# eduard-permyakov/permafrost-engine

Hardware: AMD Instinct MI355X
Metric: agent-steps/sec (+ flow-field cells/sec), every chunk field rebuilt + every agent stepped per tick (higher is better)
Workload: dtype u64-bitmask/u8 fields, f32 agents (f64 exp); 1 GPU; BASELINE configs[2]: 1024x1024 cells, 64 flow fields = 16384 chunk fields, 100000 agents; map_chunks=16, flow_fields=64, agents=100000, hz=20, dynamic_obstacles=0, parallelism=requests by destination + uid slabs x1, 1 all-gather (16 B/agent) per tick, ranks=1, rccl_ranks=1, backend=none, tile_exchange=auto, requests=reference planner fixture, has_dest_los=device lookup, initial_velocities=flow aligned, fields_ahead=True, tick_driver=c (navhip_tick_run), library=libnavhip.so (in-tree)

## Files before the change

permafrost-engine_amd/csrc/field_kernels.hip:

```cpp
#include "navhip_internal.h"

#include "wave_bits.h"

__device__ __forceinline__ bool req_uses_bfs(const nh_map_view &map, const navhip_field_req &rq,
                                             int force_generic)
{
    if(force_generic) return false;
    if(rq.type == NAVHIP_TARGET_NEAREST_PATHABLE || (rq.flags & NAVHIP_REQ_ISLAND_NEAREST)) return false;
    const nh_layer_view &L = map.layers[rq.layer];
    return L.unit_cost[(int)rq.chunk_r * map.w + rq.chunk_c] != 0;
}

__device__ __forceinline__ uint16_t portal_first_iid(const uint16_t *li, int r0, int c0, int r1, int c1)
{
    for(int r = r0; r <= r1; r++)
        for(int c = c0; c <= c1; c++) {
            const uint16_t v = li[r * 64 + c];
            if(v != NAVHIP_ISLAND_NONE) return v;
        }
    return NAVHIP_ISLAND_NONE;
}

__device__ __forceinline__ bool req_prepare(const nh_map_view &map, navhip_field_req &rq)
{
    const nh_layer_view &L = map.layers[rq.layer];
    const bool portal = rq.type == NAVHIP_TARGET_PORTAL;
    if((rq.flags & NAVHIP_REQ_IF_CHANGED) && L.changed) {
        bool ch = L.changed[(int)rq.chunk_r * map.w + rq.chunk_c] != 0;
        if(portal) ch |= L.changed[(int)rq.next_chunk_r * map.w + rq.next_chunk_c] != 0;
        if(rq.faction_id != NAVHIP_FACTION_ID_NONE && L.fac_changed)
            ch |= (L.fac_changed[(int)rq.chunk_r * map.w + rq.chunk_c] & ~rq.enemies & 0x7fff) != 0;
        if(!ch) return false;
    }
    if((rq.flags & NAVHIP_REQ_LIVE_IIDS) && portal && L.local_islands) {
        rq.port_iid = portal_first_iid(L.local_islands + ((size_t)((int)rq.chunk_r * map.w + rq.chunk_c) << 12),
                                       rq.port_r0, rq.port_c0, rq.port_r1, rq.port_c1);
        rq.next_iid = portal_first_iid(L.local_islands + ((size_t)((int)rq.next_chunk_r * map.w + rq.next_chunk_c) << 12),
                                       rq.next_r0, rq.next_c0, rq.next_r1, rq.next_c1);
        if(rq.port_iid == NAVHIP_ISLAND_NONE || rq.next_iid == NAVHIP_ISLAND_NONE) return false;
    }
    return true;
}

__device__ __forceinline__ bool next_tile_matches(const nh_map_view &map, const navhip_field_req &rq,
                                                  int gr, int gc)
{
    if(gr < 0 || gc < 0) return false;
    int cr2 = gr >> 6, cc2 = gc >> 6, r2 = gr & 63, c2 = gc & 63;
    if(cr2 != rq.next_chunk_r || cc2 != rq.next_chunk_c) return false;
    if(cr2 >= map.h || cc2 >= map.w) return false;
    if(r2 < rq.next_r0 || r2 > rq.next_r1 || c2 < rq.next_c0 || c2 > rq.next_c1) return false;
    const uint16_t *li = map.layers[rq.layer].local_islands;
    return li[((size_t)(cr2 * map.w + cc2) << 12) + r2 * 64 + c2] == rq.next_iid;
}

__device__ __forceinline__ bool portal_seed(const nh_map_view &map, const navhip_field_req &rq,
                                            int r, int c, bool passable)
{
    if(!passable) return false;
    if(r < rq.port_r0 || r > rq.port_r1 || c < rq.port_c0 || c > rq.port_c1) return false;
    const uint16_t *li = map.layers[rq.layer].local_islands;
    size_t cbase = (size_t)((int)rq.chunk_r * map.w + rq.chunk_c) << 12;
    if(rq.port_iid != NAVHIP_ISLAND_NONE && li[cbase + r * 64 + c] != rq.port_iid) return false;
    int gr = rq.chunk_r * 64 + r, gc = rq.chunk_c * 64 + c;
    return next_tile_matches(map, rq, gr - 1, gc) || next_tile_matches(map, rq, gr + 1, gc)
        || next_tile_matches(map, rq, gr, gc - 1) || next_tile_matches(map, rq, gr, gc + 1);
}

__device__ __forceinline__ uint32_t portal_fix_dir(const navhip_field_req &rq)
{
    if(rq.next_chunk_r < rq.chunk_r) return NAVHIP_FD_N;
    if(rq.next_chunk_r > rq.chunk_r) return NAVHIP_FD_S;
    if(rq.next_chunk_c < rq.chunk_c) return NAVHIP_FD_W;
    return NAVHIP_FD_E;
}

__global__ __launch_bounds__(256) void k_derive(const uint8_t *cost, const uint16_t *blockers,
                                                uint64_t *passmask, uint64_t *probemask, uint8_t *unit_cost,
                                                const uint8_t *factions, uint64_t *facmask, uint16_t *facany,
                                                const uint32_t *chunk_list, int n)
{
    int wave = (blockIdx.x * 256 + threadIdx.x) >> 6;
    int lane = threadIdx.x & 63;
    if(wave >= n) return;
    uint32_t chunk = chunk_list ? chunk_list[wave] : (uint32_t)wave;
    const uint8_t  *cb = cost + ((size_t)chunk << 12);
    const uint16_t *bl = blockers ? blockers + ((size_t)chunk << 12) : nullptr;
    uint64_t mine = 0, path = 0, blocked = 0;
    bool nonunit = false;
    for(int r = 0; r < 64; r++) {
        uint32_t cst = cb[r * 64 + lane];
        uint32_t blk = bl ? bl[r * 64 + lane] : 0;
        uint64_t m = __ballot(cst != NAVHIP_COST_IMPASSABLE && blk == 0);
        uint64_t mp = __ballot(cst != NAVHIP_COST_IMPASSABLE), mb = __ballot(blk > 0);
        nonunit |= (cst != NAVHIP_COST_IMPASSABLE && cst != 1);
        if(lane == r) { mine = m; path = mp; blocked = mb; }
    }
    passmask[(size_t)chunk * 64 + lane] = mine;
    probemask[((size_t)chunk * 64 + lane) * 2]     = path;
    probemask[((size_t)chunk * 64 + lane) * 2 + 1] = blocked;
    bool any_nonunit = __any(nonunit);
    if(lane == 0) unit_cost[chunk] = any_nonunit ? 0 : 1;
    if(factions) {
        const uint8_t *fa = factions + ((size_t)chunk * NAVHIP_MAX_FACTIONS << 12) + lane * 64;
        uint32_t any = 0;
        for(int f = 0; f < NAVHIP_MAX_FACTIONS; f++) {
            const uint64_t m = nz_row_mask(fa + ((size_t)f << 12));
            facmask[((size_t)chunk * NAVHIP_MAX_FACTIONS + f) * 64 + lane] = m;
            if(__ballot(m != 0)) any |= 1u << f;
        }
        if(lane == 0) facany[chunk] = (uint16_t)any;
    }
}

void nh_launch_derive(navhip_ctx *ctx, int layer, const uint32_t *d_chunk_list, int n, hipStream_t s)
{
    navhip_layer &L = ctx->layers[layer];
    int blocks = (n + 3) / 4;
    hipLaunchKernelGGL(k_derive, dim3(blocks), dim3(256), 0, s, L.cost, L.blockers, L.passmask, L.probemask,
                       L.unit_cost, L.factions, L.facmask, L.facany, d_chunk_list, n);
}

__device__ __forceinline__ uint64_t faction_pass_row(const nh_layer_view &L, int chunk, int lane, uint32_t enemies)
{
    const uint64_t *pm = L.probemask + ((size_t)chunk * 64 + lane) * 2;
    const uint64_t path = pm[0], blocked = pm[1];
    if(!L.facmask) return path;
    uint64_t friends = 0;
    uint32_t fs = __builtin_amdgcn_readfirstlane((int)(L.facany[chunk] & ~enemies & ((1u << NAVHIP_MAX_FACTIONS) - 1u)));
    const uint64_t *fm = L.facmask + (size_t)chunk * NAVHIP_MAX_FACTIONS * 64 + lane;
    while(fs) {
        const int f = __builtin_ctz(fs);
        fs &= fs - 1;
        friends |= fm[f * 64];
    }
    return path & ~(blocked & friends);
}

#define NH_MAXP 12
#define BFS_WAVES 4

template <bool WANT_INTEG>
__global__ __launch_bounds__(BFS_WAVES * 64) void k_field_bfs(nh_map_view map, const navhip_field_req *reqs,
                                                   int n, uint8_t *dirs, float *integ,
                                                   int force_generic, int32_t *gen_list, int gen_slot,
                                                   const int32_t *out_slot)
{
    __shared__ __attribute__((aligned(16))) uint8_t stage[BFS_WAVES][NH_CELLS];

    const int wib  = threadIdx.x >> 6;
    const int wave = blockIdx.x * BFS_WAVES + wib;
    const int lane = threadIdx.x & 63;
    if(wave >= n) return;

    navhip_field_req rq = reqs[wave];
    if(!req_uses_bfs(map, rq, force_generic)) {
        if(lane == 0) gen_list[2 + atomicAdd(&gen_list[gen_slot], 1)] = wave;
        return;
    }
    if(!req_prepare(map, rq)) return;

    const nh_layer_view &L = map.layers[rq.layer];
    const int chunk = (int)rq.chunk_r * map.w + rq.chunk_c;
    const u64x pass = mk(rq.faction_id == NAVHIP_FACTION_ID_NONE ? L.passmask[(size_t)chunk * 64 + lane]
                                                                 : faction_pass_row(L, chunk, lane, rq.enemies));

    u64x seeds = u64x{0, 0};
    if(rq.type == NAVHIP_TARGET_TILE) {
        if(lane == rq.tile_r) seeds = mk(1ull << rq.tile_c) & pass;
    }else{
        if(rq.port_c0 == rq.port_c1) {
            bool s = portal_seed(map, rq, lane, rq.port_c0, (to64(pass) >> rq.port_c0) & 1);
            if(s) seeds = mk(1ull << rq.port_c0);
        }else{
            for(int r = rq.port_r0; r <= rq.port_r1; r++) {
                uint64_t prow = __shfl(to64(pass), r);
                bool s = portal_seed(map, rq, r, lane, (prow >> lane) & 1);
                uint64_t m = __ballot(s);
                if(lane == r) seeds = mk(m);
            }
        }
    }

    u64x open = andn(pass, seeds);
    u64x frontier = seeds;
    u64x pl[NH_MAXP];
#pragma unroll
    for(int k = 0; k < NH_MAXP; k++) pl[k] = u64x{0, 0};

    int level = 0;
#define NH_BFS_LEVEL(NLOW)                                                                   \
    {                                                                                        \
        u64x nw = bfs_reach(frontier, open);                                                 \
        if(!__any(nz(nw))) break;                                                            \
        level++;                                                                             \
        pl[0] = pl[0] ^ open;                                                                \
        if(NLOW > 1) pl[1] = pl[1] ^ open;                                                   \
        if(NLOW > 2) pl[2] = pl[2] ^ open;                                                   \
        if(NLOW > 3) {                                                                       \
            const int tz = __builtin_ctz(level);          \
            _Pragma("unroll")                                                                \
            for(int k = 3; k < NH_MAXP; k++) {                                               \
                if(k <= tz) pl[k] = pl[k] ^ open;                                            \
            }                                                                                \
        }                                                                                    \
        open = andn(open, nw);                                                               \
        frontier = nw;                                                                       \
    }
    for(;;) {
        NH_BFS_LEVEL(1) NH_BFS_LEVEL(2) NH_BFS_LEVEL(1) NH_BFS_LEVEL(3)
        NH_BFS_LEVEL(1) NH_BFS_LEVEL(2) NH_BFS_LEVEL(1) NH_BFS_LEVEL(4)
    }
#undef NH_BFS_LEVEL
    const u64x reach = andn(pass, open);
#pragma unroll
    for(int k = 0; k < NH_MAXP; k++) pl[k] = pl[k] & reach;

    const int P = 32 - __builtin_clz((unsigned)level + 1);

    if(WANT_INTEG) {
        float *out = integ + ((size_t)wave << 12);
        for(int c = 0; c < 64; c++) {
            uint32_t d = 0;
#pragma unroll
            for(int k = 0; k < NH_MAXP; k++) d |= (uint32_t)((to64(pl[k]) >> c) & 1) << k;
            bool fin = (to64(reach) >> c) & 1;
            out[lane * 64 + c] = fin ? (float)d : __builtin_inff();
        }
    }

    u64x anybit = u64x{0, 0};
#pragma unroll
    for(int k = 0; k < NH_MAXP; k++) anybit = anybit | pl[k];
    const u64x zero = andn(reach, anybit);
    const u64x act  = reach & anybit;

    const u64x rN = from_n(reach), rS = from_s(reach), rW = from_w(reach), rE = from_e(reach);
    u64x eqN, eqS, eqW, eqE;
    {
        const u64x m0 = pl[0], m1 = pl[1];
        u64x n0, n1;
        n0 = from_n(pl[0]); n1 = from_n(pl[1]); eqN = andn(n0 ^ m0, n1 ^ n0 ^ m1) & rN;
        n0 = from_s(pl[0]); n1 = from_s(pl[1]); eqS = andn(n0 ^ m0, n1 ^ n0 ^ m1) & rS;
        n0 = from_w(pl[0]); n1 = from_w(pl[1]); eqW = andn(n0 ^ m0, n1 ^ n0 ^ m1) & rW;
        n0 = from_e(pl[0]); n1 = from_e(pl[1]); eqE = andn(n0 ^ m0, n1 ^ n0 ^ m1) & rE;
    }

    u64x neNW = u64x{0, 0}, neNE = neNW, neSW = neNW, neSE = neNW;
    {
        u64x b1 = u64x{~0u, ~0u};
        u64x b2 = u64x{~0u, ~0u};
#pragma unroll
        for(int k = 0; k < NH_MAXP; k++) {
            if(k < P) {
                u64x e = pl[k] ^ b1;  b1 = andn(b1, pl[k]);
                u64x f = e ^ b2;      b2 = andn(b2, e);
                u64x up = from_n(pl[k]), dn = from_s(pl[k]);
                neNW = neNW | (from_w(up) ^ f);
                neNE = neNE | (from_e(up) ^ f);
                neSW = neSW | (from_w(dn) ^ f);
                neSE = neSE | (from_e(dn) ^ f);
            }
        }
    }
    const u64x eqNW = andn(from_w(rN), neNW), eqNE = andn(from_e(rN), neNE);
    const u64x eqSW = andn(from_w(rS), neSW), eqSE = andn(from_e(rS), neSE);

    const u64x hasD = (eqNW & rN & rW) | (eqNE & rN & rE) | (eqSW & rS & rW) | (eqSE & rS & rE);
    const u64x h = act & hasD;
    const u64x g = andn(act, hasD);

    const u64x mN  = g & eqN;
    const u64x mS  = andn(g & eqS, eqN);
    const u64x mE  = andn(g & eqE, eqN | eqS);
    const u64x mW  = andn(g & eqW, eqN | eqS | eqE);
    const u64x mNW = h & eqNW;
    const u64x mNE = andn(h & eqNE, eqNW);
    const u64x mSW = andn(h & eqSW, eqNW | eqNE);
    const u64x mSE = andn(h & eqSE, eqNW | eqNE | eqSW);

    u64x D0 = mNW | mNE | mE | mS;
    u64x D1 = mN | mNE | mSW | mS;
    u64x D2 = mW | mE | mSW | mS;
    u64x D3 = mSE;
    if(rq.type == NAVHIP_TARGET_PORTAL) {
        uint32_t fd = portal_fix_dir(rq);
        if(fd & 1) D0 = D0 | zero;
        if(fd & 2) D1 = D1 | zero;
        if(fd & 4) D2 = D2 | zero;
    }

    uint8_t *out = dirs + ((size_t)(out_slot ? out_slot[wave] : wave) << 12);
    uint8_t *st = stage[wib];
    const bool inout = (rq.flags & NAVHIP_REQ_INOUT) != 0;
    if(inout) {
#pragma unroll
        for(int j = 0; j < 4; j++)
            *(uint4*)(st + j * 1024 + lane * 16) = *(const uint4*)(out + j * 1024 + lane * 16);
    }
    __builtin_amdgcn_wave_barrier();
    {
        uint32_t *row = (uint32_t*)(st + lane * 64);
        const uint64_t d0 = to64(D0), d1 = to64(D1), d2 = to64(D2), d3 = to64(D3);
        const uint64_t rc = to64(reach);
#pragma unroll
        for(int j = 0; j < 16; j++) {
            uint32_t b0 = (((uint32_t)(d0 >> (4 * j)) & 0xf) * 0x00204081u) & 0x01010101u;
            uint32_t b1 = (((uint32_t)(d1 >> (4 * j)) & 0xf) * 0x00204081u) & 0x01010101u;
            uint32_t b2 = (((uint32_t)(d2 >> (4 * j)) & 0xf) * 0x00204081u) & 0x01010101u;
            uint32_t b3 = (((uint32_t)(d3 >> (4 * j)) & 0xf) * 0x00204081u) & 0x01010101u;
            uint32_t v = b0 | (b1 << 1) | (b2 << 2) | (b3 << 3);
            if(inout) {
                uint32_t rm = ((((uint32_t)(rc >> (4 * j)) & 0xf) * 0x00204081u) & 0x01010101u) * 0xffu;
                v = (v & rm) | (row[j] & ~rm);
            }
            row[j] = v;
        }
    }
    __builtin_amdgcn_wave_barrier();
#pragma unroll
    for(int j = 0; j < 4; j++)
        *(uint4*)(out + j * 1024 + lane * 16) = *(const uint4*)(st + j * 1024 + lane * 16);
}

struct generic_lds {
    uint32_t dist[NH_CELLS];
    __attribute__((aligned(16))) uint8_t pc[NH_CELLS];
    uint8_t raw[NH_CELLS];
    uint8_t fl[NH_CELLS];
    int s_list[128], s_dmin[128], s_nlist, s_D;
};

__device__ void field_generic_one(generic_lds &S, const nh_map_view &map, const navhip_field_req *reqs,
                                  int ri, uint8_t *dirs, float *integ, int force_generic,
                                  const int32_t *out_slot)
{
    uint32_t (&dist)[NH_CELLS] = S.dist;
    uint8_t (&pc)[NH_CELLS] = S.pc;
    uint8_t (&raw)[NH_CELLS] = S.raw;
    uint8_t (&fl)[NH_CELLS] = S.fl;
    int (&s_list)[128] = S.s_list;
    int (&s_dmin)[128] = S.s_dmin;
    int &s_nlist = S.s_nlist, &s_D = S.s_D;

    const int t = threadIdx.x;
    navhip_field_req rq = reqs[ri];
    if(req_uses_bfs(map, rq, force_generic)) return;
    if(!req_prepare(map, rq)) return;

    const nh_layer_view &L = map.layers[rq.layer];
    const size_t cbase = (size_t)((int)rq.chunk_r * map.w + rq.chunk_c) << 12;
    const bool faction = rq.faction_id != NAVHIP_FACTION_ID_NONE;
    const bool modeA = rq.type == NAVHIP_TARGET_NEAREST_PATHABLE;
    const bool modeB = !modeA && (rq.flags & NAVHIP_REQ_ISLAND_NEAREST) != 0;

#pragma unroll 4
    for(int k = 0; k < 16; k++) {
        int i = k * 256 + t;
        uint32_t cst = L.cost[cbase + i];
        uint32_t blk = L.blockers ? L.blockers[cbase + i] : 0;
        bool passable;
        if(cst == NAVHIP_COST_IMPASSABLE) {
            passable = false;
        }else if(!faction) {
            passable = (blk == 0);
        }else{
            bool enemies_only = true;
            if(L.factions) {
                const uint8_t *fp = L.factions + cbase * NAVHIP_MAX_FACTIONS + i;
                for(int f = 0; f < NAVHIP_MAX_FACTIONS; f++) {
                    if(fp[(size_t)f << 12] && !(rq.enemies & (1u << f))) { enemies_only = false; break; }
                }
            }
            passable = enemies_only || (blk == 0);
        }
        pc[i] = passable ? (uint8_t)cst : (uint8_t)NAVHIP_COST_IMPASSABLE;
        raw[i] = (uint8_t)cst;
        fl[i] = (cst != NAVHIP_COST_IMPASSABLE && blk == 0) ? 1 : 0;
        dist[i] = NH_INF_U32;
    }
    if(t == 0) { s_nlist = 0; s_D = 0x7fffffff; }
    if(t < 128) s_dmin[t] = 0x7fffffff;
    __syncthreads();

    if(modeA) {
        const int start = rq.tile_r * 64 + rq.tile_c;
        if(t == 0) fl[start] |= 2;
        __syncthreads();
        if(!(fl[start] & 1)) {
            for(;;) {
                int changed = 0;
#pragma unroll 4
                for(int k = 0; k < 16; k++) {
                    int i = k * 256 + t;
                    if(fl[i] & 3) continue;
                    int r = i >> 6, c = i & 63;
                    bool nb = (r > 0 && (fl[i - 64] & 2)) || (r < 63 && (fl[i + 64] & 2))
                           || (c > 0 && (fl[i - 1] & 2)) || (c < 63 && (fl[i + 1] & 2));
                    if(nb) { fl[i] |= 2; changed = 1; }
                }
                if(!__syncthreads_or(changed)) break;
            }
#pragma unroll 4
            for(int k = 0; k < 16; k++) {
                int i = k * 256 + t;
                if(!(fl[i] & 1)) continue;
                int r = i >> 6, c = i & 63;
                bool nb = (r > 0 && (fl[i - 64] & 2)) || (r < 63 && (fl[i + 64] & 2))
                       || (c > 0 && (fl[i - 1] & 2)) || (c < 63 && (fl[i + 1] & 2));
                if(nb) dist[i] = 0;
            }
        }else if(t == 0) {
            dist[start] = 0;
        }
        __syncthreads();
        for(;;) {
            int changed = 0;
#pragma unroll 4
            for(int k = 0; k < 16; k++) {
                int i = k * 256 + t;
                if(fl[i] & 1) continue;
                int r = i >> 6, c = i & 63;
                uint32_t m = NH_INF_U32;
                if(r > 0)  m = min(m, dist[i - 64]);
                if(r < 63) m = min(m, dist[i + 64]);
                if(c > 0)  m = min(m, dist[i - 1]);
                if(c < 63) m = min(m, dist[i + 1]);
                if(m < NH_INF_U32) {
                    uint32_t nd = m + raw[i];
                    if(nd < dist[i]) { dist[i] = nd; changed = 1; }
                }
            }
            if(!__syncthreads_or(changed)) break;
        }
    }else{
        if(rq.type == NAVHIP_TARGET_TILE) {
            if(t == 0) {
                int i = rq.tile_r * 64 + rq.tile_c;
                if(pc[i] != NAVHIP_COST_IMPASSABLE) {
                    if(modeB) s_list[s_nlist++] = i; else dist[i] = 0;
                }
            }
        }else{
            int nr = rq.port_r1 - rq.port_r0 + 1, nc = rq.port_c1 - rq.port_c0 + 1;
            for(int j = t; j < nr * nc; j += 256) {
                int r = rq.port_r0 + j / nc, c = rq.port_c0 + j % nc;
                if(portal_seed(map, rq, r, c, pc[r * 64 + c] != NAVHIP_COST_IMPASSABLE)) {
                    if(modeB) { int p = atomicAdd(&s_nlist, 1); if(p < 128) s_list[p] = r * 64 + c; }
                    else dist[r * 64 + c] = 0;
                }
            }
        }
        __syncthreads();
        if(modeB) {
            if(t == 0 && s_nlist == 0 && rq.type == NAVHIP_TARGET_TILE)
                s_list[s_nlist++] = rq.tile_r * 64 + rq.tile_c;
            __syncthreads();
            const int nl = min(s_nlist, 128);
            const uint16_t *li = L.local_islands + cbase;
            const uint16_t *gi = L.islands ? L.islands + cbase : nullptr;
            const uint32_t want = rq.aux_iid;
            for(int q = 0; q < nl; q++) {
                const int f = s_list[q], fr = f >> 6, fc = f & 63;
                const uint32_t giid = gi ? gi[f] : NAVHIP_ISLAND_NONE;
                int best = 0x7fffffff;
#pragma unroll 4
                for(int k = 0; k < 16; k++) {
                    int i = k * 256 + t;
                    if(!(fl[i] & 1)) continue;
                    if(want != NAVHIP_ISLAND_NONE && li[i] != want) continue;
                    if(giid != NAVHIP_ISLAND_NONE && gi[i] != giid) continue;
                    int d = abs((i >> 6) - fr) + abs((i & 63) - fc);
                    best = min(best, d);
                }
                if(best < 0x7fffffff) atomicMin(&s_dmin[q], best);
            }
            __syncthreads();
            if(t == 0) {
                int D = 0x7fffffff;
                for(int q = 0; q < nl; q++) D = min(D, s_dmin[q]);
                s_D = D;
            }
            __syncthreads();
            const int D = s_D;
            if(D < 0x7fffffff) {
                for(int q = 0; q < nl; q++) {
                    if(s_dmin[q] != D) continue;
                    const int f = s_list[q], fr = f >> 6, fc = f & 63;
                    const uint32_t giid = gi ? gi[f] : NAVHIP_ISLAND_NONE;
#pragma unroll 4
                    for(int k = 0; k < 16; k++) {
                        int i = k * 256 + t;
                        if(!(fl[i] & 1)) continue;
                        if(want != NAVHIP_ISLAND_NONE && li[i] != want) continue;
                        if(giid != NAVHIP_ISLAND_NONE && gi[i] != giid) continue;
                        if(abs((i >> 6) - fr) + abs((i & 63) - fc) == D) dist[i] = 0;
                    }
                }
            }
            __syncthreads();
        }

        for(;;) {
            int changed = 0;
#pragma unroll 4
            for(int k = 0; k < 16; k++) {
                int i = k * 256 + t;
                uint32_t cst = pc[i];
                if(cst == NAVHIP_COST_IMPASSABLE) continue;
                int r = i >> 6, c = i & 63;
                uint32_t m = NH_INF_U32;
                if(r > 0)  m = min(m, dist[i - 64]);
                if(r < 63) m = min(m, dist[i + 64]);
                if(c > 0)  m = min(m, dist[i - 1]);
                if(c < 63) m = min(m, dist[i + 1]);
                if(m < NH_INF_U32) {
                    uint32_t nd = m + cst;
                    if(nd < dist[i]) { dist[i] = nd; changed = 1; }
                }
            }
            if(!__syncthreads_or(changed)) break;
        }
    }

    const bool inout = (rq.flags & NAVHIP_REQ_INOUT) != 0 || modeA || modeB;
    uint8_t *out = dirs + ((size_t)(out_slot ? out_slot[ri] : ri) << 12);
    const uint32_t fixdir = (rq.type == NAVHIP_TARGET_PORTAL) ? portal_fix_dir(rq) : NAVHIP_FD_NONE;
    uint8_t res[16];
#pragma unroll 4
    for(int k = 0; k < 16; k++) {
        int i = k * 256 + t;
        int r = i >> 6, c = i & 63;
        uint32_t d = dist[i];
        uint32_t dir;
        if(d >= NH_INF_U32) {
            dir = inout ? out[i] : NAVHIP_FD_NONE;
        }else if(d == 0) {
            dir = modeA ? out[i] : fixdir;
        }else{
            const uint32_t I = NH_INF_U32;
            uint32_t dn = r > 0  ? dist[i - 64] : I, ds = r < 63 ? dist[i + 64] : I;
            uint32_t dw = c > 0  ? dist[i - 1]  : I, de = c < 63 ? dist[i + 1]  : I;
            uint32_t dnw = (r > 0  && c > 0)  ? dist[i - 65] : I;
            uint32_t dne = (r > 0  && c < 63) ? dist[i - 63] : I;
            uint32_t dsw = (r < 63 && c > 0)  ? dist[i + 63] : I;
            uint32_t dse = (r < 63 && c < 63) ? dist[i + 65] : I;
            uint32_t mc = min(min(dn, ds), min(dw, de));
            if(dn < I && dw < I) mc = min(mc, dnw);
            if(dn < I && de < I) mc = min(mc, dne);
            if(ds < I && dw < I) mc = min(mc, dsw);
            if(ds < I && de < I) mc = min(mc, dse);
            if(dn == mc)       dir = NAVHIP_FD_N;
            else if(ds == mc)  dir = NAVHIP_FD_S;
            else if(de == mc)  dir = NAVHIP_FD_E;
            else if(dw == mc)  dir = NAVHIP_FD_W;
            else if(dnw == mc) dir = NAVHIP_FD_NW;
            else if(dne == mc) dir = NAVHIP_FD_NE;
            else if(dsw == mc) dir = NAVHIP_FD_SW;
            else               dir = NAVHIP_FD_SE;
        }
        res[k] = (uint8_t)dir;
        if(integ) integ[((size_t)ri << 12) + i] = (d >= NH_INF_U32) ? __builtin_inff() : (float)d;
    }
    __syncthreads();
#pragma unroll
    for(int k = 0; k < 16; k++) pc[k * 256 + t] = res[k];
    __syncthreads();
    *(uint4*)(out + t * 16) = *(const uint4*)(pc + t * 16);
}

__global__ __launch_bounds__(256) void k_field_generic(nh_map_view map, const navhip_field_req *reqs,
                                                       int n, uint8_t *dirs, float *integ,
                                                       int force_generic, int32_t *gen_list, int gen_slot,
                                                       const int32_t *out_slot)
{
    __shared__ generic_lds S;
    const int count = gen_list ? gen_list[gen_slot] : n;
    if(gen_list && blockIdx.x == 0 && threadIdx.x == 0) gen_list[gen_slot ^ 1] = 0;
    for(int w = blockIdx.x; w < count; w += gridDim.x) {
        const int ri = gen_list ? gen_list[2 + w] : w;
        field_generic_one(S, map, reqs, ri, dirs, integ, force_generic, out_slot);
        __syncthreads();
    }
}

int nh_launch_fields(navhip_ctx *ctx, const navhip_field_req *d_reqs, int n, uint8_t *d_dirs,
                     float *d_integ, int32_t *d_gen_list, hipStream_t s, const int32_t *d_out_slot)
{
    nh_map_view mv;
    nh_fill_map_view(ctx, &mv);
    const int force_generic = ctx->field_kernel_mode == 1;
    const int gen_slot = force_generic ? 0 : (int)(ctx->gen_launches++ & 1);
    if(!force_generic) {
        dim3 grid((n + BFS_WAVES - 1) / BFS_WAVES);
        if(d_integ)
            hipLaunchKernelGGL(k_field_bfs<true>, grid, dim3(BFS_WAVES * 64), 0, s, mv, d_reqs, n, d_dirs,
                               d_integ, force_generic, d_gen_list, gen_slot, d_out_slot);
        else
            hipLaunchKernelGGL(k_field_bfs<false>, grid, dim3(BFS_WAVES * 64), 0, s, mv, d_reqs, n, d_dirs,
                               d_integ, force_generic, d_gen_list, gen_slot, d_out_slot);
    }
    bool heavy = force_generic;
    for(int l = 0; l < NAVHIP_NAV_LAYER_MAX; l++) heavy = heavy || (ctx->layers[l].cost && ctx->layers[l].nonunit_costs);
    const int gmax = heavy ? 2048 : 512;
    hipLaunchKernelGGL(k_field_generic, dim3(n < gmax ? n : gmax), dim3(256), 0, s, mv, d_reqs, n, d_dirs,
                       d_integ, force_generic, force_generic ? (int32_t*)nullptr : d_gen_list, gen_slot, d_out_slot);
    return force_generic ? -1 : gen_slot;
}
```

permafrost-engine_amd/csrc/wave_bits.h:

```cpp
#pragma once
#include <hip/hip_runtime.h>
#include <stdint.h>

struct u64x { uint32_t lo, hi; };

__device__ __forceinline__ u64x mk(uint64_t v) { return u64x{(uint32_t)v, (uint32_t)(v >> 32)}; }
__device__ __forceinline__ uint64_t to64(u64x v) { return ((uint64_t)v.hi << 32) | v.lo; }
__device__ __forceinline__ u64x operator|(u64x a, u64x b) { return u64x{a.lo | b.lo, a.hi | b.hi}; }
__device__ __forceinline__ u64x operator&(u64x a, u64x b) { return u64x{a.lo & b.lo, a.hi & b.hi}; }
__device__ __forceinline__ u64x operator^(u64x a, u64x b) { return u64x{a.lo ^ b.lo, a.hi ^ b.hi}; }
__device__ __forceinline__ u64x operator~(u64x a) { return u64x{~a.lo, ~a.hi}; }
__device__ __forceinline__ bool nz(u64x a) { return (a.lo | a.hi) != 0; }
__device__ __forceinline__ u64x andn(u64x a, u64x b) { return u64x{a.lo & ~b.lo, a.hi & ~b.hi}; }

__device__ __forceinline__ u64x from_w(u64x v)
{
    return u64x{v.lo << 1, __builtin_amdgcn_alignbit(v.hi, v.lo, 31)};
}
__device__ __forceinline__ u64x from_e(u64x v)
{
    return u64x{__builtin_amdgcn_alignbit(v.hi, v.lo, 1), v.hi >> 1};
}
__device__ __forceinline__ u64x from_n(u64x v)
{
    return u64x{(uint32_t)__builtin_amdgcn_update_dpp(0, (int)v.lo, 0x138, 0xf, 0xf, true),
                (uint32_t)__builtin_amdgcn_update_dpp(0, (int)v.hi, 0x138, 0xf, 0xf, true)};
}
__device__ __forceinline__ u64x from_s(u64x v)
{
    return u64x{(uint32_t)__builtin_amdgcn_update_dpp(0, (int)v.lo, 0x130, 0xf, 0xf, true),
                (uint32_t)__builtin_amdgcn_update_dpp(0, (int)v.hi, 0x130, 0xf, 0xf, true)};
}

#ifdef NH_HOSTSIM
__device__ __forceinline__ uint32_t nh_keep32(uint32_t x) { return x; }
#else
__device__ __forceinline__ uint32_t nh_keep32(uint32_t x) { asm volatile("" : "+v"(x)); return x; }
#endif
__device__ __forceinline__ u64x bfs_reach(u64x f, u64x open)
{
    const u64x w = from_w(f), e = from_e(f), n = from_n(f), s = from_s(f);
    const uint32_t a0 = nh_keep32(w.lo | n.lo), a1 = nh_keep32(w.hi | n.hi);
    const uint32_t b0 = nh_keep32(e.lo | s.lo), b1 = nh_keep32(e.hi | s.hi);
    return u64x{(a0 | b0) & open.lo, (a1 | b1) & open.hi};
}

__device__ __forceinline__ uint32_t nz_bytes4(uint32_t w)
{
    const uint32_t top = (((w & 0x7f7f7f7fu) + 0x7f7f7f7fu) | w) & 0x80808080u;
    return (((top >> 7) * 0x00204081u) >> 21) & 0xfu;
}
__device__ __forceinline__ uint64_t nz_row_mask(const uint8_t *row)
{
    uint64_t m = 0;
#pragma unroll
    for(int j = 0; j < 4; j++) {
        const uint4 q = *(const uint4*)(row + j * 16);
        const uint32_t n = nz_bytes4(q.x) | (nz_bytes4(q.y) << 4) | (nz_bytes4(q.z) << 8) | (nz_bytes4(q.w) << 12);
        m |= (uint64_t)n << (16 * j);
    }
    return m;
}
```

Measured before the change: 39.19 million agent-steps/s.

## Batch BFS termination checks, skip high-plane diagonal work, bit-transpose direction output

The BFS loop now checks for an empty frontier once per block of eight unrolled levels instead of after every level. Extra levels run on empty frontiers and do no harm because open stops changing. The diagonal inequality loop over the high distance planes now runs only when some active cell has a diagonal neighbour reachable while both adjacent orthogonals are not; otherwise only the low three planes are processed. The per-nibble multiply expansion that packs four direction bitplanes into bytes is replaced by a shuffle-and-perm bit transpose with 128-bit LDS writes. This trims ALU work per chunk field, at the cost of up to seven wasted BFS levels and a subtle correctness condition on the wide test.

```diff
diff --git a/permafrost-engine_amd/csrc/field_kernels.hip b/permafrost-engine_amd/csrc/field_kernels.hip
--- a/permafrost-engine_amd/csrc/field_kernels.hip
+++ b/permafrost-engine_amd/csrc/field_kernels.hip
@@ -192,7 +192,6 @@
 #define NH_BFS_LEVEL(NLOW)                                                                   \
     {                                                                                        \
         u64x nw = bfs_reach(frontier, open);                                                 \
-        if(!__any(nz(nw))) break;                                                            \
         level++;                                                                             \
         pl[0] = pl[0] ^ open;                                                                \
         if(NLOW > 1) pl[1] = pl[1] ^ open;                                                   \
@@ -201,16 +200,18 @@
             const int tz = __builtin_ctz(level);          \
             _Pragma("unroll")                                                                \
             for(int k = 3; k < NH_MAXP; k++) {                                               \
-                if(k <= tz) pl[k] = pl[k] ^ open;                                            \
+                 \
+                 \
+                if(k <= tz) { asm volatile(""); pl[k] = pl[k] ^ open; }                      \
             }                                                                                \
         }                                                                                    \
         open = andn(open, nw);                                                               \
         frontier = nw;                                                                       \
     }
-    for(;;) {
+    do {
         NH_BFS_LEVEL(1) NH_BFS_LEVEL(2) NH_BFS_LEVEL(1) NH_BFS_LEVEL(3)
         NH_BFS_LEVEL(1) NH_BFS_LEVEL(2) NH_BFS_LEVEL(1) NH_BFS_LEVEL(4)
-    }
+    } while(__any(nz(frontier)));
 #undef NH_BFS_LEVEL
     const u64x reach = andn(pass, open);
 #pragma unroll
@@ -246,13 +247,19 @@
         n0 = from_e(pl[0]); n1 = from_e(pl[1]); eqE = andn(n0 ^ m0, n1 ^ n0 ^ m1) & rE;
     }
 
+    bool wide;
+    {
+        const u64x rNW = from_w(rN), rNE = from_e(rN), rSW = from_w(rS), rSE = from_e(rS);
+        const u64x behind = act & (andn(rNW, rN | rW) | andn(rNE, rN | rE) | andn(rSW, rS | rW) | andn(rSE, rS | rE));
+        wide = __any(nz(behind));
+    }
     u64x neNW = u64x{0, 0}, neNE = neNW, neSW = neNW, neSE = neNW;
     {
         u64x b1 = u64x{~0u, ~0u};
         u64x b2 = u64x{~0u, ~0u};
 #pragma unroll
         for(int k = 0; k < NH_MAXP; k++) {
-            if(k < P) {
+            if(k < 3 || (wide && k < P)) {
                 u64x e = pl[k] ^ b1;  b1 = andn(b1, pl[k]);
                 u64x f = e ^ b2;      b2 = andn(b2, e);
                 u64x up = from_n(pl[k]), dn = from_s(pl[k]);
@@ -300,21 +307,26 @@
     }
     __builtin_amdgcn_wave_barrier();
     {
-        uint32_t *row = (uint32_t*)(st + lane * 64);
-        const uint64_t d0 = to64(D0), d1 = to64(D1), d2 = to64(D2), d3 = to64(D3);
-        const uint64_t rc = to64(reach);
-#pragma unroll
-        for(int j = 0; j < 16; j++) {
-            uint32_t b0 = (((uint32_t)(d0 >> (4 * j)) & 0xf) * 0x00204081u) & 0x01010101u;
-            uint32_t b1 = (((uint32_t)(d1 >> (4 * j)) & 0xf) * 0x00204081u) & 0x01010101u;
-            uint32_t b2 = (((uint32_t)(d2 >> (4 * j)) & 0xf) * 0x00204081u) & 0x01010101u;
-            uint32_t b3 = (((uint32_t)(d3 >> (4 * j)) & 0xf) * 0x00204081u) & 0x01010101u;
-            uint32_t v = b0 | (b1 << 1) | (b2 << 2) | (b3 << 3);
+        uint4 *row = (uint4*)(st + lane * 64);
+        const uint32_t d0[2] = {D0.lo, D0.hi}, d1[2] = {D1.lo, D1.hi}, d2[2] = {D2.lo, D2.hi}, d3[2] = {D3.lo, D3.hi};
+        const uint32_t rc[2] = {reach.lo, reach.hi};
+#pragma unroll
+        for(int hf = 0; hf < 2; hf++) {
+            uint32_t v[8];
+            planes_to_bytes32(d0[hf], d1[hf], d2[hf], d3[hf], v);
             if(inout) {
-                uint32_t rm = ((((uint32_t)(rc >> (4 * j)) & 0xf) * 0x00204081u) & 0x01010101u) * 0xffu;
-                v = (v & rm) | (row[j] & ~rm);
-            }
-            row[j] = v;
+                uint32_t rm[8];
+                planes_to_bytes32(rc[hf], rc[hf], rc[hf], rc[hf], rm);
+                const uint4 o0 = row[2 * hf], o1 = row[2 * hf + 1];
+                const uint32_t o[8] = {o0.x, o0.y, o0.z, o0.w, o1.x, o1.y, o1.z, o1.w};
+#pragma unroll
+                for(int i = 0; i < 8; i++) {
+                    const uint32_t m = rm[i] | (rm[i] << 4);
+                    v[i] = (v[i] & m) | (o[i] & ~m);
+                }
+            }
+            row[2 * hf]     = uint4{v[0], v[1], v[2], v[3]};
+            row[2 * hf + 1] = uint4{v[4], v[5], v[6], v[7]};
         }
     }
     __builtin_amdgcn_wave_barrier();
diff --git a/permafrost-engine_amd/csrc/wave_bits.h b/permafrost-engine_amd/csrc/wave_bits.h
--- a/permafrost-engine_amd/csrc/wave_bits.h
+++ b/permafrost-engine_amd/csrc/wave_bits.h
@@ -45,6 +45,36 @@
     return u64x{(a0 | b0) & open.lo, (a1 | b1) & open.hi};
 }
 
+#ifdef NH_HOSTSIM
+__device__ __forceinline__ uint32_t nh_perm(uint32_t hi, uint32_t lo, uint32_t sel)
+{
+    const uint64_t pair = ((uint64_t)hi << 32) | lo;
+    uint32_t r = 0;
+    for(int i = 0; i < 4; i++) r |= (uint32_t)((pair >> (8 * ((sel >> (8 * i)) & 7))) & 0xff) << (8 * i);
+    return r;
+}
+#else
+__device__ __forceinline__ uint32_t nh_perm(uint32_t hi, uint32_t lo, uint32_t sel) { return __builtin_amdgcn_perm(hi, lo, sel); }
+#endif
+
+__device__ __forceinline__ void planes_to_bytes32(uint32_t p0, uint32_t p1, uint32_t p2, uint32_t p3, uint32_t *y)
+{
+    const uint32_t m1 = 0x55555555u, m2 = 0x33333333u, m4 = 0x0f0f0f0fu;
+    const uint32_t a0 = (p0 & m1) | ((p1 << 1) & ~m1), a1 = ((p0 >> 1) & m1) | (p1 & ~m1);
+    const uint32_t b0 = (p2 & m1) | ((p3 << 1) & ~m1), b1 = ((p2 >> 1) & m1) | (p3 & ~m1);
+    const uint32_t w0 = (a0 & m2) | ((b0 << 2) & ~m2), w2 = ((a0 >> 2) & m2) | (b0 & ~m2);
+    const uint32_t w1 = (a1 & m2) | ((b1 << 2) & ~m2), w3 = ((a1 >> 2) & m2) | (b1 & ~m2);
+    const uint32_t t0 = nh_perm(w1, w0, 0x05010400u), t1 = nh_perm(w1, w0, 0x07030602u);
+    const uint32_t t2 = nh_perm(w3, w2, 0x05010400u), t3 = nh_perm(w3, w2, 0x07030602u);
+    const uint32_t v[4] = {nh_perm(t2, t0, 0x05040100u), nh_perm(t2, t0, 0x07060302u),
+                           nh_perm(t3, t1, 0x05040100u), nh_perm(t3, t1, 0x07060302u)};
+#pragma unroll
+    for(int k = 0; k < 4; k++) {
+        y[2 * k]     = v[k] & m4;
+        y[2 * k + 1] = (v[k] >> 4) & m4;
+    }
+}
+
 __device__ __forceinline__ uint32_t nz_bytes4(uint32_t w)
 {
     const uint32_t top = (((w & 0x7f7f7f7fu) + 0x7f7f7f7fu) | w) & 0x80808080u;
```

Result: faster. 39.60 million agent-steps/s, median of 6 (+1.1%).
